# DavidSevic/gpu-nbody-simulation

Hardware: AMD Instinct MI355X
Metric: body-steps/sec (higher is better)
Workload: dtype f32

## Files before the change

### gpu-nbody-simulation_amd/csrc/bh_engine.hip

```cpp
#include "../../include/bhgpu.h"

#include <hip/hip_runtime.h>

#include <algorithm>
#include <cmath>
#include <cstdio>
#include <cstdlib>
#include <cstring>
#include <string>
#include <type_traits>
#include <vector>

#include "bh_tree.hpp"
#include "bh_walk_exact.hpp"
#include "bh_walk_f64.hpp"
#include "bh_diag.hpp"
#include "bh_direct.hpp"
#include "bh_init.hpp"
#include "bh_let.hpp"
#include "bh_migrate.hpp"
#include "bh_walk_fast.h"

using namespace bh;

#ifdef BHGPU_EXPERIMENTS
#include "../../scripts/experiments/bh_engine_hooks.hpp"
#else
struct ExpHooks {
    hipError_t create(int64_t) { return hipSuccess; }
    void walk_args(WalkFastArgs &) const {}
    void destroy(int64_t) {}
};
#endif

namespace {

thread_local std::string g_create_error;

struct DevBuf {
    void *p = nullptr;
    size_t bytes = 0;
};

}

struct bh_ctx {
    bh_config cfg{};
    int Dm = 0;
    enum class Mode { Exact, F64, Mixed, F32 };
    Mode mode = Mode::Exact;
    bool tree64() const { return mode == Mode::Exact || mode == Mode::F64; }
    bool state64() const { return mode != Mode::F32; }
    bool compat = true;
    bool exact_thresholds = false;
    int device = 0;
    hipStream_t stream = nullptr;
    bool own_stream = false;
    int64_t n = 0;
    bool uploaded = false, tree_valid = false;
    int64_t internal_cap = 0, node_cap = 0;
    int64_t bfs_max = 12288;
    int exact_bpw = 0;
    int walk_split = 0;
    bool walk_asm = true;
    int sort_bucket = 1;
    bool last_sort_bucket = false, last_sort_packed = false;
    int64_t samples_n = -1;
    uint64_t *splitters = nullptr;
    uint16_t *sort_dig = nullptr;
    int build_items = 0;
    bool hilbert = false;
    int partial_count = 0;
    double *bslots = nullptr;
    bool slots_valid = false;
    bool slots_dirty = true;

    void *pos = nullptr, *vel = nullptr, *mass = nullptr, *force = nullptr;
    void *pos2 = nullptr, *vel2 = nullptr, *mass2 = nullptr, *force2 = nullptr;
    uint32_t *orig = nullptr, *orig2 = nullptr;
    bool orig_identity = true;
    int reorder_every = 16;
    int64_t builds = 0;
    float2 *spos = nullptr;
    float4 *sstate = nullptr;
    float *smass = nullptr;
    uint64_t *keys[2] = {nullptr, nullptr};
    uint32_t *vals[2] = {nullptr, nullptr};
    uint64_t *keys_sorted = nullptr;
    uint32_t *perm = nullptr;
    uint32_t *radix_counts = nullptr, *bsum_sort = nullptr, *bsum_u32 = nullptr, *cnt = nullptr;
    uint64_t *coarse = nullptr;
    uint32_t *cell_first = nullptr;
    d3 *terms = nullptr, *bsum_d3 = nullptr;
    double *partial = nullptr, *box = nullptr;
    NodeD *gd = nullptr;
    LinkD *ld = nullptr;
    QuadF *qf = nullptr;
    NodeAux *aux = nullptr;
    int32_t *self_node = nullptr, *cell_depth = nullptr;
    uint32_t *com_pending = nullptr;
    TreeCounters *ctr = nullptr;

    int rank = 0, world = 1;
    bool let_mode = false, external_box = false;
    int64_t let_cap = 0, quads_local = 0;
    int64_t forest_base = 0;
    uint64_t *needmask = nullptr;
    uint32_t *let_tsum = nullptr, *let_outidx = nullptr;
    QuadF *let_send = nullptr;
    double *lbounds = nullptr, *all_bounds = nullptr;
    float2 *acc_part = nullptr;
    LetCounters *let_ctr = nullptr;
    int64_t *gid = nullptr;
    uint32_t *group_cost = nullptr;
    const void **walk_consts = nullptr;
    bool aux_full = false;
    bool group_cost_valid = false;
    uint32_t *body_counts = nullptr;
    double *phi = nullptr;
    uint32_t *phi_counts = nullptr;
    double *diag_part = nullptr, *diag_out = nullptr, *slots_save = nullptr;
    bool phi_current = false;
    uint32_t *slot_of = nullptr;
    int64_t *direct_targets = nullptr;
    double2 *direct_out = nullptr;
    void *check_force = nullptr;
    uint32_t *check_counts = nullptr, *check_cost = nullptr;
    TreeCounters *ctr_save = nullptr;
    bool sort_pack = true;
    unsigned long long *orb_hist = nullptr;
    double *mig_send = nullptr, *mig_recv = nullptr;
    ExpHooks exp;

    std::vector<hipEvent_t> ev;
    hipEvent_t ev_step[2] = {nullptr, nullptr}, ev_build[2] = {nullptr, nullptr};
    hipEvent_t ev_grp[3] = {nullptr, nullptr, nullptr};
    hipEvent_t ev_let[3] = {nullptr, nullptr, nullptr};
    bool let_timed = false;
    bool time_groups = false;
    int64_t steps_done = 0;
    int32_t last_nsteps = 0;
    int timed_pairs = 0;
    int64_t walk_launches = 0;
    bool step_timed = false;

    std::vector<void *> allocs;
    uint64_t device_bytes = 0;
    std::string err;
};

using Mode = bh_ctx::Mode;

namespace {

int fail(bh_ctx *c, int code, const std::string &msg)
{
    if (c) c->err = msg; else g_create_error = msg;
    return code;
}

#define BH_HIP(c, call)                                                                         \
    do {                                                                                        \
        hipError_t e_ = (call);                                                                 \
        if (e_ != hipSuccess)                                                                   \
            return fail((c), BH_ERR_DEVICE,                                                     \
                        std::string(#call) + ": " + hipGetErrorString(e_));                     \
    } while (0)

template <typename T>
int dev_alloc(bh_ctx *c, T **out, size_t count)
{
    void *p = nullptr;
    const size_t bytes = std::max<size_t>(count, 1) * sizeof(T);
    hipError_t e = hipMalloc(&p, bytes);
    if (e != hipSuccess)
        return fail(c, BH_ERR_DEVICE, std::string("hipMalloc(") + std::to_string(bytes) + "): " + hipGetErrorString(e));
    c->allocs.push_back(p);
    c->device_bytes += bytes;
    *out = static_cast<T *>(p);
    return BH_OK;
}

inline void dev_free(bh_ctx *c, void *p)
{
    if (!p) return;
    auto it = std::find(c->allocs.begin(), c->allocs.end(), p);
    if (it != c->allocs.end()) { c->allocs.erase(it); (void)hipFree(p); }
}

inline unsigned blocks_for(int64_t n, int per_block) { return (unsigned)((n + per_block - 1) / per_block); }

template <typename F>
void dispatch(F &&f) { f(); }
template <typename F, typename... B>
void dispatch(F &&f, bool b, B... rest)
{
    if (b) dispatch([&](auto... t) { f(std::true_type{}, t...); }, rest...);
    else dispatch([&](auto... t) { f(std::false_type{}, t...); }, rest...);
}

inline int64_t cell_span(const bh_ctx *c)
{
    return std::max<int64_t>(1, std::min<int64_t>(c->internal_cap, std::max<int64_t>(c->n - 1, 0) * (int64_t)std::max(1, c->Dm)));
}

void owned_range(const bh_ctx *c, int64_t *lo, int64_t *hi)
{
    if (c->let_mode) { *lo = 0; *hi = c->n; return; }
    const int64_t per = (c->n + c->world - 1) / c->world;
    const int64_t chunk = (per + kBlock - 1) / kBlock * kBlock;
    *lo = std::min<int64_t>(c->n, chunk * c->rank);
    *hi = std::min<int64_t>(c->n, chunk * (c->rank + 1));
}

constexpr int64_t kComClimbMaxBodies = 32768;
constexpr int64_t kSmallBuildBodies = 327680;
constexpr int64_t kMediumBuildBodies = 786432;
constexpr int kSmallItems = 2;

template <typename Real2, typename Real>
__global__ __launch_bounds__(kBlock) void reorder_state_kernel(uint32_t *__restrict__ perm, const Real2 *__restrict__ pos,
                                                                const Real2 *__restrict__ vel, const Real *__restrict__ mass,
                                                                const float2 *__restrict__ acc, const uint32_t *__restrict__ orig,
                                                                Real2 *__restrict__ pos2, Real2 *__restrict__ vel2,
                                                                Real *__restrict__ mass2, float2 *__restrict__ acc2,
                                                                uint32_t *__restrict__ orig2, int64_t n)
{
    const int64_t s = (int64_t)blockIdx.x * kBlock + threadIdx.x;
    if (s >= n) return;
    const uint32_t b = perm[s];
    pos2[s] = pos[b]; vel2[s] = vel[b]; mass2[s] = mass[b]; acc2[s] = acc[b];
    orig2[s] = orig ? orig[b] : b;
    perm[s] = (uint32_t)s;
}

static void launch_nodes_fast(bh_ctx *c, bool full_aux, hipStream_t st)
{
    dispatch([&](auto compat, auto full) {
        hipLaunchKernelGGL((nodes_fast_kernel<decltype(compat)::value, decltype(full)::value>), dim3(blocks_for(cell_span(c), kBlock)),
                           dim3(kBlock), 0, st, c->keys_sorted, c->coarse, c->cnt, c->cell_first, c->spos, c->smass, c->box,
                           c->terms, c->n, c->Dm, c->cfg.theta, c->internal_cap, c->qf, c->aux, c->ctr);
    }, c->compat, full_aux);
    c->aux_full = full_aux;
}

void clean_slots(bh_ctx *c)
{
    if (c->slots_dirty) hipLaunchKernelGGL(bounds_slots_reset, dim3(1), dim3(kWave), 0, c->stream, c->bslots);
    c->slots_dirty = true;
}

template <bool TREE64, bool STATE64 = TREE64, int ITEMS = kItems>
int enqueue_build_t(bh_ctx *c)
{
    constexpr int TILE = kBlock * ITEMS;
    static_assert(!TREE64 || STATE64, "an fp64 tree is built from fp64 state");
    using Real2 = typename std::conditional<STATE64, double2, float2>::type;
    using Real = typename std::conditional<STATE64, double, float>::type;
    const int64_t n = c->n;
    const int Dm = c->Dm;
    hipStream_t st = c->stream;
    const Real2 *pos = static_cast<const Real2 *>(c->pos);
    const Real *mass = static_cast<const Real *>(c->mass);

    const bool from_walk = c->slots_valid;
    double *slots = c->external_box ? nullptr : c->bslots;
    if (slots) {
        if (!from_walk) {
            const unsigned nbb = std::max(1u, std::min(1024u, blocks_for(n, kBlock)));
            clean_slots(c);
            hipLaunchKernelGGL((bounds_partial<Real2>), dim3(nbb), dim3(kBlock), 0, st, pos, n, slots);
        }
        c->slots_valid = false;
        if (n > 0) c->slots_dirty = false;
    }

    if (n > 0) {
        const bool pack = Dm >= 1 && 2 * Dm <= kPackShift && n <= ((int64_t)1 << (64 - kPackShift))
                          && c->sort_pack;
        const bool single = pack && n >= 2 && n <= 4 * kBsThreads && c->sort_bucket == 1;
        const bool bucket = !single && pack && n >= 2 && n <= kBucketMaxNBig && (c->sort_bucket == 2 || (c->sort_bucket == 1 && c->samples_n == n));
        const int nb = (n <= kBucketMaxN) ? kBuckets : kBucketsBig;
        const int ns = (nb == kBuckets) ? ((n > (int64_t)1 << 18) ? 2 * kBuckets : kBuckets)
                                        : ((n > (int64_t)3 << 20) ? kMaxSplitSamples : kBucketsBig);
        static_assert(kBucketMaxN == (int64_t)1 << 20 && kBucketMaxNBig == (int64_t)1 << 22, "BASELINE configs 3 and 4 fit");
        c->last_sort_bucket = bucket || single; c->last_sort_packed = pack;
        {
            const unsigned nkb = blocks_for(n, kBlock);
            auto keys_launch = [&](auto fs, auto pk, auto hil) {
                constexpr bool H = decltype(hil)::value, P = decltype(pk)::value, F = decltype(fs)::value;
                const bool smp = P && bucket;
                hipLaunchKernelGGL((keys_kernel<Real2, H, P, F>), dim3(nkb + (smp ? ns / kWave : 0)), dim3(kBlock), 0, st, pos, c->box,
                                   c->keys[0], c->vals[0], n, Dm, (smp && !TREE64) ? (const float2 *)c->spos : nullptr, c->splitters, nb, ns,
                                   slots, c->ctr, smp ? c->bsum_sort : nullptr, smp ? nb : 0, (smp && TREE64) ? c->perm : nullptr,
                                   from_walk ? 1 : 0);
            };
            dispatch(keys_launch, slots != nullptr, pack, c->hilbert);
        }
        if (c->time_groups) (void)hipEventRecord(c->ev_grp[0], st);
        const unsigned nbl = blocks_for(n, ITEMS == kItems ? kSortTile : TILE);
        int cur = 0;
        if (single) {
            hipLaunchKernelGGL(bucket_sort_kernel, dim3(1), dim3(kBsThreads), 0, st, c->keys[0], c->keys[1], c->vals[1],
                               nullptr, nullptr, &c->ctr->sort_spills, &c->ctr->sort_reruns, (int)n);
            cur = 1;
        } else if (bucket) {
            constexpr int SI = (ITEMS == kItems ? kSortItems : ITEMS);
            auto pass = [&](auto bits_tag) {
                constexpr int NBITS = decltype(bits_tag)::value;
                if constexpr (TREE64) {
                    hipLaunchKernelGGL((radix_hist<SI, NBITS, true>), dim3(nbl), dim3(kBlock), 0, st, c->keys[0], c->radix_counts, n,
                                       0, (int)nbl, c->splitters, c->sort_dig, nullptr);
                    hipLaunchKernelGGL(radix_rowscan, dim3(1 << NBITS), dim3(kBlock), 0, st, c->radix_counts, c->bsum_sort, (int)nbl);
                    hipLaunchKernelGGL((radix_scatter_w<SI, NBITS, 1, true, false>), dim3(nbl), dim3(kBlock), 0, st, c->keys[0], c->vals[0],
                                       c->keys[1], c->vals[1], c->radix_counts, c->bsum_sort, n, 0, (int)nbl, c->sort_dig,
                                       c->bsum_sort + kBucketStartOffset);
                } else {
                    hipLaunchKernelGGL((radix_hist<SI, NBITS, true>), dim3(nbl), dim3(kBlock), 0, st, c->keys[0], c->radix_counts, n,
                                       0, (int)nbl, c->splitters, c->sort_dig, c->bsum_sort);
                    hipLaunchKernelGGL((radix_scatter_w<SI, NBITS, 1, true>), dim3(nbl), dim3(kBlock), 0, st, c->keys[0], c->vals[0],
                                       c->keys[1], c->vals[1], c->radix_counts, c->bsum_sort, n, 0, (int)nbl, c->sort_dig,
                                       c->bsum_sort + kBucketStartOffset);
                }
            };
            if (nb == kBuckets) pass(std::integral_constant<int, 8>{}); else pass(std::integral_constant<int, 10>{});
            hipLaunchKernelGGL(bucket_sort_kernel, dim3(nb), dim3(kBsThreads), 0, st, c->keys[1], c->keys[0], c->vals[0],
                               c->bsum_sort, c->bsum_sort + kBucketStartOffset, &c->ctr->sort_spills, &c->ctr->sort_reruns, 0);
            cur = 0;
        } else {
            constexpr int SB = kSortBits, SR = 1 << SB, SI = (ITEMS == kItems ? kSortItems : ITEMS);
            const int passes = (2 * Dm + SB - 1) / SB;
            for (int p = 0; p < passes; ++p) {
                const int shift = p * SB;
                hipLaunchKernelGGL((radix_hist<SI, SB>), dim3(nbl), dim3(kBlock), 0, st, c->keys[cur], c->radix_counts, n,
                                   shift, (int)nbl);
                hipLaunchKernelGGL(radix_rowscan, dim3(SR), dim3(kBlock), 0, st, c->radix_counts, c->bsum_sort, (int)nbl);
                if (pack && p + 1 < passes)
                    hipLaunchKernelGGL((radix_scatter_w<SI, SB, 1>), dim3(nbl), dim3(kBlock), 0, st, c->keys[cur], c->vals[cur],
                                       c->keys[cur ^ 1], c->vals[cur ^ 1], c->radix_counts, c->bsum_sort, n, shift, (int)nbl);
                else if (pack)
                    hipLaunchKernelGGL((radix_scatter_w<SI, SB, 2>), dim3(nbl), dim3(kBlock), 0, st, c->keys[cur], c->vals[cur],
                                       c->keys[cur ^ 1], c->vals[cur ^ 1], c->radix_counts, c->bsum_sort, n, shift, (int)nbl);
                else
                    hipLaunchKernelGGL((radix_scatter_w<SI, SB>), dim3(nbl), dim3(kBlock), 0, st, c->keys[cur], c->vals[cur],
                                       c->keys[cur ^ 1], c->vals[cur ^ 1], c->radix_counts, c->bsum_sort, n, shift,
                                       (int)nbl);
                cur ^= 1;
            }
        }
        c->keys_sorted = c->keys[cur];
        c->perm = c->vals[cur];
        if constexpr (!TREE64) {
            if (c->reorder_every > 0 && c->builds % c->reorder_every == 0) {
                hipLaunchKernelGGL((reorder_state_kernel<Real2, Real>), dim3(blocks_for(n, kBlock)), dim3(kBlock), 0, st,
                                   c->perm, pos, static_cast<const Real2 *>(c->vel), mass,
                                   static_cast<const float2 *>(c->force), c->orig_identity ? nullptr : c->orig,
                                   static_cast<Real2 *>(c->pos2), static_cast<Real2 *>(c->vel2),
                                   static_cast<Real *>(c->mass2), static_cast<float2 *>(c->force2), c->orig2, n);
                std::swap(c->pos, c->pos2); std::swap(c->vel, c->vel2); std::swap(c->mass, c->mass2);
                std::swap(c->force, c->force2); std::swap(c->orig, c->orig2);
                c->orig_identity = false;
                pos = static_cast<const Real2 *>(c->pos);
                mass = static_cast<const Real *>(c->mass);
            }
        }
        c->builds += 1;
        if (c->time_groups) (void)hipEventRecord(c->ev_grp[1], st);

        using SReal2 = typename std::conditional<TREE64, double2, float2>::type;
        using SReal = typename std::conditional<TREE64, double, float>::type;
        auto scan_part = [&](auto si_tag) {
            constexpr int SI = decltype(si_tag)::value;
            const unsigned nbs = blocks_for(n + 1, kBlock * SI);
            hipLaunchKernelGGL((prep_kernel<TREE64, SI, Real2, Real, SReal2, SReal>), dim3(nbs), dim3(kBlock), 0, st,
                               c->keys_sorted, c->perm, pos, mass, c->cnt, c->bsum_u32, (SReal2 *)c->spos,
                               (SReal *)c->smass, c->terms, c->bsum_d3, c->coarse, n, Dm, slots);
            constexpr bool TSRC = !TREE64 && std::is_same<Real2, SReal2>::value;
            if (nbs <= 8u * kBlock) {
                hipLaunchKernelGGL((scan_apply2<TREE64, SI, true, TSRC>), dim3(nbs), dim3(kBlock), 0, st, c->cnt, c->bsum_u32,
                                   c->terms, c->bsum_d3, (int)nbs, n, c->cell_first, c->internal_cap, c->ctr,
                                   (const float2 *)c->spos, (const float *)c->smass);
            } else {
                hipLaunchKernelGGL(scan_top2, dim3(TREE64 ? 1 : 2), dim3(kBlock), 0, st, c->bsum_u32, c->bsum_d3,
                                   (int)nbs, c->ctr);
                hipLaunchKernelGGL((scan_apply2<TREE64, SI, false, TSRC>), dim3(nbs), dim3(kBlock), 0, st, c->cnt, c->bsum_u32,
                                   c->terms, c->bsum_d3, (int)nbs, n, c->cell_first, c->internal_cap, c->ctr,
                                   (const float2 *)c->spos, (const float *)c->smass);
            }
        };
        if (ITEMS == kItems && n <= (int64_t)1 << 21) scan_part(std::integral_constant<int, 4>{});
        else scan_part(std::integral_constant<int, ITEMS>{});
        c->samples_n = n;
        if (c->time_groups) (void)hipEventRecord(c->ev_grp[2], st);
    } else {
        if (slots)
            hipLaunchKernelGGL((keys_kernel<Real2, false, false, true>), dim3(1), dim3(kBlock), 0, st, pos, c->box, c->keys[0],
                               c->vals[0], n, Dm, nullptr, nullptr, 0, 0, slots, c->ctr);
        c->keys_sorted = c->keys[0];
        c->perm = c->vals[0];
        if (c->time_groups) for (auto e : c->ev_grp) (void)hipEventRecord(e, st);
    }

    if constexpr (TREE64) {
        hipLaunchKernelGGL(nodes_exact_kernel, dim3(blocks_for(cell_span(c), kBlock)), dim3(kBlock), 0, st, c->keys_sorted, c->perm,
                           c->cnt, c->cell_first, pos, mass, c->box, n, Dm, c->internal_cap, c->gd, c->ld, c->self_node,
                           c->cell_depth, c->com_pending, c->ctr, (c->mode == Mode::F64 || c->exact_thresholds) ? c->cfg.theta : 0.0,
                           c->exact_thresholds ? 1 : 0);
    } else {
        launch_nodes_fast(c, false, st);
    }
    if (TREE64 && n > 1 && c->internal_cap > 0) {
        const int64_t span = cell_span(c);
        if (n <= kComClimbMaxBodies) {
            hipLaunchKernelGGL(com_up_kernel, dim3(blocks_for(span, kBlock)), dim3(kBlock), 0, st, c->gd, c->ld,
                               c->self_node, c->com_pending, c->ctr, c->internal_cap);
        } else {
            for (int d = Dm - 1; d >= 0; --d)
                hipLaunchKernelGGL(com_level_kernel, dim3(blocks_for(span, kBlock)), dim3(kBlock), 0, st, c->gd,
                                   c->self_node, c->cell_depth, c->ctr, c->internal_cap, d);
        }
    }
    BH_HIP(c, hipGetLastError());
    c->tree_valid = true;
    return BH_OK;
}

template <int ITEMS>
static int enqueue_build_items(bh_ctx *c)
{
    if (c->tree64()) return enqueue_build_t<true, true, ITEMS>(c);
    return c->state64() ? enqueue_build_t<false, true, ITEMS>(c) : enqueue_build_t<false, false, ITEMS>(c);
}

int enqueue_build(bh_ctx *c)
{
    int items = c->build_items;
    if (items == 0) items = c->n <= kSmallBuildBodies ? 2 : c->n <= kMediumBuildBodies ? 4 : 8;
    if (c->n > (1 << 22)) items = 8;
    switch (items) {
    case 2: return enqueue_build_items<2>(c);
    case 4: return enqueue_build_items<4>(c);
    default: return enqueue_build_items<kItems>(c);
    }
}

static int fp64_bodies_per_wave(const bh_ctx *c, int64_t cnt)
{
    if (c->mode == Mode::F64 && (c->cfg.flags & BH_FLAG_WALK_NO_SPLIT)) return kWave;
    int b = 1;
    if (c->exact_bpw > 0) b = c->exact_bpw;
    else if (c->mode == Mode::F64) {
        while (b < kWave && (int64_t)b * 4096 < cnt) b <<= 1;
    } else if (cnt > 4096) {
        b = 16;
        while (b < kWave && (int64_t)b * 2048 < cnt) b <<= 1;
    }
// ... 172 lines not shown
}

int check_overflow(bh_ctx *c)
{
    TreeCounters h{};
    BH_HIP(c, hipMemcpyAsync(&h, c->ctr, sizeof(h), hipMemcpyDeviceToHost, c->stream));
    BH_HIP(c, hipStreamSynchronize(c->stream));
    if (h.overflow || (int64_t)h.n_internal > c->internal_cap)
        return fail(c, BH_ERR_CAPACITY, "tree needs " + std::to_string(1 + 4 * (int64_t)h.n_internal) +
                                        " nodes, node_capacity is " + std::to_string(c->node_cap));
    return BH_OK;
}

int new_bodies(bh_ctx *c, int64_t n)
{
    c->n = n;
    c->partial_count = 0; c->slots_valid = false;
    c->samples_n = -1;
    c->uploaded = true;
    c->tree_valid = false;
    c->steps_done = 0;
    c->orig_identity = true;
    c->builds = 0;
    c->group_cost_valid = false;
    c->phi_current = false;
    if (c->gid && n > 0) {
        hipLaunchKernelGGL(iota_i64_kernel, dim3(blocks_for(n, kBlock)), dim3(kBlock), 0, c->stream, c->gid, n);
        BH_HIP(c, hipGetLastError());
    }
    return BH_OK;
}

}

static int download_pairs(bh_ctx *c, const void *dev, double *host, int64_t count, bool is64);
static int to_caller_order(bh_ctx *c, double *host, int per);

extern "C" {

int bh_abi_version(void) { return BHGPU_ABI_VERSION; }

#ifndef BHGPU_BUILD_INFO
#define BHGPU_BUILD_INFO "digest=unknown flags=unknown"
#endif
const char *bh_build_info(void) { return BHGPU_BUILD_INFO; }

const char *bh_last_error(const bh_ctx *ctx) { return ctx ? ctx->err.c_str() : g_create_error.c_str(); }

int bh_create(const bh_config *cfg, bh_ctx **out)
{
    if (!cfg || !out) return fail(nullptr, BH_ERR_ARG, "bh_create: null argument");
    *out = nullptr;
    if (cfg->capacity < 0 || cfg->capacity > 0x7fffffffLL - 8)
        return fail(nullptr, BH_ERR_ARG, "bh_create: capacity out of range");
    if (cfg->max_depth < 1 || cfg->max_depth > 32)
        return fail(nullptr, BH_ERR_ARG, "bh_create: max_depth must be 1..32");
    if (!(cfg->theta > 0.0)) return fail(nullptr, BH_ERR_ARG, "bh_create: theta must be > 0");
    if (cfg->precision != BH_PRECISION_F64_EXACT && cfg->precision != BH_PRECISION_F32 &&
        cfg->precision != BH_PRECISION_MIXED && cfg->precision != BH_PRECISION_F64)
        return fail(nullptr, BH_ERR_ARG, "bh_create: unknown precision");
    int ndev = 0;
    if (hipGetDeviceCount(&ndev) != hipSuccess || ndev <= 0)
        return fail(nullptr, BH_ERR_NO_DEVICE, "bh_create: no HIP device (libbhgpu has no CPU fallback)");
    if (cfg->device < 0 || cfg->device >= ndev)
        return fail(nullptr, BH_ERR_ARG, "bh_create: device ordinal out of range");

    bh_ctx *c = new bh_ctx();
    c->cfg = *cfg;
    c->Dm = cfg->max_depth - 1;
    c->mode = cfg->precision == BH_PRECISION_F64_EXACT ? Mode::Exact
            : cfg->precision == BH_PRECISION_F64       ? Mode::F64
            : cfg->precision == BH_PRECISION_MIXED     ? Mode::Mixed : Mode::F32;
    c->compat = cfg->reference_compat != 0;
    c->device = cfg->device;
    if (const char *e = std::getenv("BH_WALK_SPLIT")) c->walk_split = std::atoi(e);
    if (const char *e = std::getenv("BH_EXACT_BPW")) { const int b = std::atoi(e); c->exact_bpw = (b >= 1 && b <= kWave && (b & (b - 1)) == 0) ? b : 0; }
    if (const char *e = std::getenv("BH_WALK_ASM")) c->walk_asm = std::atoi(e) != 0;
    if (const char *e = std::getenv("BH_EXACT_BFS_MAX")) c->bfs_max = std::max(0, std::atoi(e));
    c->exact_thresholds = c->mode == Mode::Exact && c->walk_asm && !(cfg->flags & BH_FLAG_WALK_PORTABLE);
    if (const char *e = std::getenv("BH_SORT_PACK")) c->sort_pack = std::atoi(e) != 0;
    if (const char *e = std::getenv("BH_SORT_BUCKET")) c->sort_bucket = std::atoi(e);
    if (const char *e = std::getenv("BH_BUILD_ITEMS")) c->build_items = std::atoi(e);
    if (const char *e = std::getenv("BH_REORDER_EVERY")) c->reorder_every = std::max(0, std::atoi(e));
    c->hilbert = !c->tree64();
    if (const char *e = std::getenv("BH_HILBERT")) c->hilbert = !c->tree64() && std::atoi(e) != 0;
    auto bail = [&](int rc) { g_create_error = c->err; bh_destroy(c); return rc; };

    if (hipSetDevice(c->device) != hipSuccess) { c->err = "hipSetDevice failed"; return bail(BH_ERR_DEVICE); }
    if (hipStreamCreateWithFlags(&c->stream, hipStreamNonBlocking) != hipSuccess) {
        c->err = "hipStreamCreate failed"; return bail(BH_ERR_DEVICE);
    }
    c->own_stream = true;

    const int64_t cap = std::max<int64_t>(cfg->capacity, 1);
    c->node_cap = cfg->node_capacity > 0 ? cfg->node_capacity : 8 * cap + 1024;
    if (c->Dm < 15) {
        int64_t full = 0, wdt = 1;
        for (int l = 0; l <= c->Dm; ++l) { full += wdt; wdt *= 4; }
        c->node_cap = std::min(c->node_cap, std::max<int64_t>(full, 1));
    }
    c->internal_cap = (c->node_cap - 1) / 4;

    const size_t rs = c->state64() ? sizeof(double) : sizeof(float);
    int rc = 0;
    auto A = [&](auto **pp, size_t count) { if (!rc) rc = dev_alloc(c, pp, count); };
    { char *t; A(&t, cap * 2 * rs); c->pos = t; }
    { char *t; A(&t, cap * 2 * rs); c->vel = t; }
    { char *t; A(&t, cap * rs); c->mass = t; }
    { char *t; A(&t, cap * 2 * (c->tree64() ? sizeof(double) : sizeof(float))); c->force = t; }
    if (!c->tree64()) {
        { char *t; A(&t, cap * 2 * rs); c->pos2 = t; }
        { char *t; A(&t, cap * 2 * rs); c->vel2 = t; }
        { char *t; A(&t, cap * rs); c->mass2 = t; }
        { char *t; A(&t, cap * 2 * sizeof(float)); c->force2 = t; }
        A(&c->orig, cap); A(&c->orig2, cap);
    }
    A(&c->keys[0], cap); A(&c->keys[1], cap); A(&c->vals[0], cap); A(&c->vals[1], cap);
    A(&c->cnt, cap + 1);
    { const size_t nbl = std::max<size_t>(blocks_for(cap, kSortTile), blocks_for(std::min<int64_t>(cap, 1 << 22), kBlock * kSmallItems));
      const size_t big = (cap > kBucketMaxN) ? (size_t)kBucketsBig * blocks_for(std::min<int64_t>(cap, kBucketMaxNBig), kBlock * kSmallItems) : 0;
      A(&c->radix_counts, std::max<size_t>((size_t)(1 << kSortBits) * nbl, big));
      A(&c->bsum_sort, 2 * kBucketStartOffset);
      A(&c->splitters, kBucketsBig);
      A(&c->sort_dig, (size_t)std::min<int64_t>(cap, kBucketMaxNBig) + 16);
    }
    const size_t scan_tiles = std::max<size_t>(blocks_for(cap + 1, kTile), blocks_for(std::min<int64_t>(cap, 1 << 22) + 1, kBlock * kSmallItems)) + 8;
    A(&c->bsum_u32, scan_tiles);
    A(&c->partial, 4 * (std::max<size_t>(1024, blocks_for(cap, kWave)) + 2));
    A(&c->box, 8); A(&c->bslots, 4 * kBoundSlots);
    A(&c->ctr, 1);
    if (c->tree64()) {
        { NodeD *g0 = nullptr; LinkD *l0 = nullptr; A(&g0, c->node_cap + 4); A(&l0, c->node_cap + 4);
          if (!rc) { c->gd = g0 + 3; c->ld = l0 + 3; } }
        A(&c->self_node, c->internal_cap + 1); A(&c->com_pending, c->internal_cap + 1); A(&c->cell_depth, c->internal_cap + 1);
        A(&c->cell_first, c->internal_cap + 1);
    } else {
        A(&c->qf, c->internal_cap + 1); A(&c->aux, 4 * (c->internal_cap + 1));
        A(&c->cell_first, c->internal_cap + 1);
        A(&c->gid, cap); A(&c->group_cost, cap / kWave + 2); A(&c->walk_consts, 4);
        A(&c->coarse, cap / 256 + 2);
        A(&c->spos, cap); A(&c->sstate, cap + 64 * kBlock + 1024); A(&c->smass, cap);
        A(&c->terms, cap + 1); A(&c->bsum_d3, scan_tiles);
    }
    if (rc) return bail(rc);
    if (hipMemset(c->ctr, 0, sizeof(TreeCounters)) != hipSuccess) { c->err = "hipMemset failed"; return bail(BH_ERR_DEVICE); }
    if (!c->tree64()) {
        const void *wc[4] = {c->aux, c->spos, c->smass, nullptr};
        if (hipMemcpy(c->walk_consts, wc, sizeof(wc), hipMemcpyHostToDevice) != hipSuccess) { c->err = "hipMemcpy failed"; return bail(BH_ERR_DEVICE); }
    }
    if (!c->tree64() && c->exp.create(cap) != hipSuccess) { c->err = "experiment hooks: allocation failed"; return bail(BH_ERR_DEVICE); }
    auto create = [](auto &evs) { for (auto &e : evs) if (hipEventCreate(&e) != hipSuccess) return false; return true; };
    if (!create(c->ev_step) || !create(c->ev_build) || !create(c->ev_grp) || !create(c->ev_let)) {
        c->err = "hipEventCreate failed"; return bail(BH_ERR_DEVICE);
    }
    *out = c;
    return BH_OK;
}

void bh_destroy(bh_ctx *c)
{
    if (!c) return;
    (void)hipSetDevice(c->device);
    if (c->stream) (void)hipStreamSynchronize(c->stream);
    c->exp.destroy(c->n);
    for (void *p : c->allocs) (void)hipFree(p);
    auto destroy = [](auto &evs) { for (auto e : evs) if (e) (void)hipEventDestroy(e); };
// ... 1058 lines not shown
```

### gpu-nbody-simulation_amd/csrc/bh_tree.hpp

```cpp
#pragma once

#include <type_traits>

#include "bh_prims.hpp"
#include "bh_sort.hpp"
#include "bh_nodes.hpp"
#include "bh_bounds.hpp"

namespace bh {

constexpr int kCoarse = 256;

__device__ __forceinline__ int shared_levels(uint64_t a, uint64_t b, int Dm)
{
    const uint64_t x = a ^ b;
    if (x == 0) return Dm;
    return (__clzll((long long)x) - (64 - 2 * Dm)) >> 1;
}

template <typename Real2>
__global__ __launch_bounds__(kBlock) void bounds_partial(const Real2 *__restrict__ pos, int64_t n, double *slots)
{
    double xlo = INFINITY, xhi = -INFINITY, ylo = INFINITY, yhi = -INFINITY;
    for (int64_t i = (int64_t)blockIdx.x * kBlock + threadIdx.x; i < n; i += (int64_t)gridDim.x * kBlock) {
// ... 46 lines not shown
            if (bx) x0 = mx; else x1 = mx;
            if (by) y0 = my; else y1 = my;
        }
    } else {
        for (int l = 0; l < Dm; ++l) {
            const double mx = (x0 + x1) / 2, my = (y0 + y1) / 2;
            const int c = pick_child(x, y, mx, my);
            if (HILBERT) {
                k = (k << 2) | (uint64_t)hilbert_digit(state, c);
                state = hilbert_next(state, c);
            } else {
                k = (k << 2) | (uint64_t)c;
            }
            descend(c, mx, my, x0, x1, y0, y1);
        }
    }
    return k;
}

__device__ __forceinline__ uint32_t hilbert3_entry(uint32_t t)
{
    int state = (int)(t >> 6);
    const uint32_t iy3 = (t >> 3) & 7u, ix3 = t & 7u;
    uint32_t digits = 0;
#pragma unroll
    for (int l = 2; l >= 0; --l) {
        const int c = (int)(((ix3 >> l) & 1u) | (((iy3 >> l) & 1u) << 1));
        digits = (digits << 2) | (uint32_t)hilbert_digit(state, c);
        state = hilbert_next(state, c);
    }
    return ((uint32_t)state << 6) | digits;
}

template <bool HILBERT>
__device__ __forceinline__ uint64_t key_of_fast(double x, double y, double x0, double x1, double y0, double y1, int Dm,
                                                double scale_x, double scale_y, double margin_x, double margin_y,
                                                const uint8_t *hil3 = nullptr)
{
    const double side = (double)(1u << Dm);
    const double tx = (x - x0) * scale_x, ty = (y - y0) * scale_y;
    const double fx = floor(tx), fy = floor(ty);
    const double rx = tx - fx, ry = ty - fy;
    const bool sure = rx > margin_x && rx < 1.0 - margin_x && ry > margin_y && ry < 1.0 - margin_y &&
                      fx >= 0.0 && fx < side && fy >= 0.0 && fy < side;
    if (!sure) return key_of<HILBERT>(x, y, x0, x1, y0, y1, Dm);
    const uint32_t ix = (uint32_t)fx, iy = (uint32_t)fy;
    uint64_t k = 0;
    int state = 0;
    int l = Dm - 1;
    if (HILBERT && hil3 != nullptr) {
        for (; (l + 1) % 3 != 0; --l) {
            const int c = (int)(((ix >> l) & 1u) | (((iy >> l) & 1u) << 1));
            k = (k << 2) | (uint64_t)hilbert_digit(state, c);
            state = hilbert_next(state, c);
        }
        uint32_t st = (uint32_t)state;
        for (; l >= 2; l -= 3) {
            const uint32_t e = hil3[(st << 6) | (((iy >> (l - 2)) & 7u) << 3) | ((ix >> (l - 2)) & 7u)];
            k = (k << 6) | (uint64_t)(e & 63u);
            st = e >> 6;
        }
        return k;
    }
    if (!HILBERT) {
        auto spread = [](uint32_t v) -> uint64_t {
            uint64_t u = v;
            u = (u | (u << 16)) & 0x0000FFFF0000FFFFull;
            u = (u | (u << 8)) & 0x00FF00FF00FF00FFull;
            u = (u | (u << 4)) & 0x0F0F0F0F0F0F0F0Full;
            u = (u | (u << 2)) & 0x3333333333333333ull;
            u = (u | (u << 1)) & 0x5555555555555555ull;
            return u;
        };
        return spread(ix) | (spread(iy) << 1);
    }
    for (; l >= 0; --l) {
        const int c = (int)(((ix >> l) & 1u) | (((iy >> l) & 1u) << 1));
        k = (k << 2) | (uint64_t)hilbert_digit(state, c);
        state = hilbert_next(state, c);
    }
    return k;
}

template <typename Real2, bool HILBERT, bool PACK = false, bool FROM_SLOTS = false>
__global__ __launch_bounds__(kBlock) void keys_kernel(const Real2 *__restrict__ pos,
                                                       double *box_global,
                                                       uint64_t *__restrict__ keys,
                                                       uint32_t *__restrict__ idx, int64_t n, int Dm,
                                                       const float2 *__restrict__ samples = nullptr,
                                                       uint64_t *__restrict__ splitters = nullptr, int nb = 0,
                                                       int ns = 0, double *slots = nullptr, TreeCounters *ctr = nullptr,
                                                       uint32_t *__restrict__ zero_words = nullptr, int n_zero = 0,
                                                       const uint32_t *__restrict__ sample_perm = nullptr, int from_walk = 0)
{
    if (blockIdx.x == 0)
        for (int k = threadIdx.x; k < n_zero; k += kBlock) zero_words[k] = 0u;
    __shared__ double s_box[FROM_SLOTS ? 8 : 1];
    __shared__ int s_keep;
    if (FROM_SLOTS) {
        if (threadIdx.x < kWave) {
            const double *sl = slots + 4 * threadIdx.x;
            const double xlo = wave_min(sl[0]), xhi = wave_max(sl[1]), ylo = wave_min(sl[2]), yhi = wave_max(sl[3]);
            const bool keep = from_walk && xlo > xhi;
            if (threadIdx.x == 0) s_keep = keep ? 1 : 0;
            if (threadIdx.x < 2) {
                const int a = threadIdx.x;
                if (keep) {
                    s_box[2 * a] = box_global[2 * a]; s_box[2 * a + 1] = box_global[2 * a + 1];
                    s_box[4 + a] = box_global[4 + a]; s_box[6 + a] = box_global[6 + a];
                } else {
                    const double ex = xhi - xlo, ey = yhi - ylo;
                    const double span = (ex < ey) ? ey : ex;
                    double pad = 0.1 * span;
                    if (span == 0.0) pad = 1e-6;
                    s_box[2 * a] = (a ? ylo : xlo) - pad; s_box[2 * a + 1] = (a ? yhi : xhi) + pad;
                    write_key_consts_axis(s_box, a, Dm);
                }
            }
        }
        __syncthreads();
        if (blockIdx.x == 0 && threadIdx.x == 0) {
            if (!s_keep) {
#pragma unroll
                for (int k = 0; k < 8; ++k) box_global[k] = s_box[k];
                ctr->overflow = 0;
            }
            ctr->n_internal = 0;
            ctr->visits = 0; ctr->interactions = 0; ctr->wave_nodes = 0; ctr->wave_quads = 0; ctr->wave_accepts = 0;
        }
    }
    double x0, x1, y0, y1, bk4, bk5, bk6, bk7;
    if (FROM_SLOTS) {
        x0 = s_box[0]; x1 = s_box[1]; y0 = s_box[2]; y1 = s_box[3]; bk4 = s_box[4]; bk5 = s_box[5]; bk6 = s_box[6]; bk7 = s_box[7];
    } else {
        x0 = box_global[0]; x1 = box_global[1]; y0 = box_global[2]; y1 = box_global[3];
        bk4 = box_global[4]; bk5 = box_global[5]; bk6 = box_global[6]; bk7 = box_global[7];
    }
    const int nsb = (samples != nullptr || sample_perm != nullptr) ? ns / kWave : 0;
    if ((int)blockIdx.x < nsb) {
        __shared__ uint64_t sk[kMaxSplitSamples];
        const int t = threadIdx.x;
        const int Ds = Dm, lg_ns = 31 - __clz(ns), lg_os = lg_ns - (31 - __clz(nb));
        const double side = (double)(1u << Ds), top = side - 1.0, down = 1.0 / (double)(1u << (Dm - Ds));
        const double sx = (bk4 > 0.0) ? bk4 * down : side / (x1 - x0), sy = (bk5 > 0.0) ? bk5 * down : side / (y1 - y0);
        float2 qs[kMaxSplitSamples / kBlock];
#pragma unroll
        for (int k = 0; k < kMaxSplitSamples / kBlock; ++k) {
            const int j = t + k * kBlock;
            qs[k] = float2{0.f, 0.f};
            if (j < ns) {
                const int64_t rk = ((int64_t)j * n) >> lg_ns;
                if (sample_perm != nullptr) { const Real2 pp = pos[sample_perm[rk]]; qs[k] = float2{(float)pp.x, (float)pp.y}; }
                else qs[k] = samples[rk];
            }
        }
#pragma unroll
        for (int k = 0; k < kMaxSplitSamples / kBlock; ++k) {
            const int j = t + k * kBlock;
            if (j >= ns) break;
            uint64_t mine = 0;
            if (j > 0) {
                const float2 q = qs[k];
                const double fx = fmin(fmax(((double)q.x - x0) * sx, 0.0), top);
                const double fy = fmin(fmax(((double)q.y - y0) * sy, 0.0), top);
                const uint32_t ix = (uint32_t)(int)fx, iy = (uint32_t)(int)fy;
                int state = 0;
                for (int l = Ds - 1; l >= 0; --l) {
                    const int cc = (int)(((ix >> l) & 1u) | (((iy >> l) & 1u) << 1));
                    mine = (mine << 2) | (uint64_t)(HILBERT ? hilbert_digit(state, cc) : cc);
                    state = hilbert_next(state, cc);
                }
            }
            sk[j] = (mine << 11) | (uint64_t)j;
        }
        __syncthreads();
        const int sidx = (int)blockIdx.x * kWave + (t >> 2), part = t & 3, span = ns >> 2;
        const uint64_t tagged = sk[sidx];
        int rank = 0;
#pragma unroll 16
        for (int q = part * span; q < (part + 1) * span; ++q) rank += (sk[q] < tagged) ? 1 : 0;
        rank += __shfl_xor(rank, 1);
        rank += __shfl_xor(rank, 2);
        if (part == 0 && (rank & ((1 << lg_os) - 1)) == 0) splitters[rank >> lg_os] = tagged >> 11;
        return;
    }
    __shared__ uint8_t s_hil3[HILBERT ? 256 : 1];
    if (HILBERT) {
        static_assert(kBlock == 256, "one table entry per thread");
        s_hil3[threadIdx.x] = (uint8_t)hilbert3_entry(threadIdx.x);
        __syncthreads();
    }
    const int64_t i = ((int64_t)blockIdx.x - nsb) * kBlock + threadIdx.x;
    if (i >= n) return;
    const uint64_t k = key_of_fast<HILBERT>((double)pos[i].x, (double)pos[i].y, x0, x1, y0, y1, Dm, bk4, bk5, bk6, bk7,
                                            HILBERT ? s_hil3 : nullptr);
    if (PACK) {
        keys[i] = k | ((uint64_t)i << kPackShift);
    } else {
        keys[i] = k;
        idx[i] = (uint32_t)i;
    }
}

template <bool EXACT, int ITEMS, typename Real2, typename Real, typename SReal2 = Real2, typename SReal = Real>
__global__ __launch_bounds__(kBlock) void prep_kernel(const uint64_t *__restrict__ keys,
                                                       const uint32_t *__restrict__ perm,
                                                       const Real2 *__restrict__ pos,
                                                       const Real *__restrict__ mass,
                                                       uint32_t *__restrict__ cnt,
                                                       uint32_t *__restrict__ bsum_u32,
                                                       SReal2 *__restrict__ spos, SReal *__restrict__ smass,
                                                       d3 *__restrict__ terms, d3 *__restrict__ bsum_d3,
                                                       uint64_t *__restrict__ coarse, int64_t n, int Dm,
                                                       double *slots_reset = nullptr)
{
    if (slots_reset != nullptr && blockIdx.x == 0 && threadIdx.x < kBoundSlots) {
        double *w = slots_reset + 4 * threadIdx.x;
        w[0] = INFINITY; w[1] = -INFINITY; w[2] = INFINITY; w[3] = -INFINITY;
    }
    __shared__ uint32_t smu[kWavesPerBlock + 1];
    __shared__ d3 smd[kWavesPerBlock + 1];
    const int64_t base = (int64_t)blockIdx.x * (kBlock * ITEMS);
    uint32_t csum = 0;
    d3 tsum{0.0, 0.0, 0.0};
#pragma unroll
    for (int k = 0; k < ITEMS; ++k) {
        const int64_t i = base + k * kBlock + threadIdx.x;
        if (i < n) {
            uint32_t c = 0;
            if (i + 1 < n) {
                const uint64_t kc = keys[i];
                const int L = shared_levels(kc, keys[i + 1], Dm);
                const int Lp = (i == 0) ? -1 : shared_levels(keys[i - 1], kc, Dm);
                const int hi = (L < Dm - 1) ? L : Dm - 1;
                c = (hi > Lp) ? (uint32_t)(hi - Lp) : 0u;
            }
            cnt[i] = c;
            csum += c;
            if (!EXACT && (i & (kCoarse - 1)) == 0) coarse[i / kCoarse] = keys[i];
            if (!EXACT) {
                const uint32_t b = perm[i];
                const Real2 p = pos[b];
                const Real m = mass[b];
                spos[i] = SReal2{static_cast<SReal>(p.x), static_cast<SReal>(p.y)};
                smass[i] = static_cast<SReal>(m);
                const d3 t{(double)m, (double)m * (double)p.x, (double)m * (double)p.y};
                if (!std::is_same<Real2, SReal2>::value) terms[i] = t;
                tsum += t;
            }
        } else if (!EXACT && i == n) {
            if (!std::is_same<Real2, SReal2>::value) terms[n] = d3{0.0, 0.0, 0.0};
        }
    }
    uint32_t utot;
    (void)block_exclusive_sum(csum, smu, utot);
    if (threadIdx.x == 0) bsum_u32[blockIdx.x] = utot;
    if (!EXACT) {
        d3 dtot;
        (void)block_exclusive_sum(tsum, smd, dtot);
        if (threadIdx.x == 0) bsum_d3[blockIdx.x] = dtot;
    }
}

__global__ __launch_bounds__(kBlock) void scan_top2(uint32_t *__restrict__ bsum_u32,
                                                     d3 *__restrict__ bsum_d3, int nb,
                                                     TreeCounters *ctr)
{
    if (blockIdx.x == 0) {
        __shared__ uint32_t sm[kWavesPerBlock + 1];
        uint32_t carry = 0;
        for (int c0 = 0; c0 < nb; c0 += kBlock) {
            const int i = c0 + threadIdx.x;
            const uint32_t v = (i < nb) ? bsum_u32[i] : 0u;
            uint32_t tot;
            const uint32_t ex = block_exclusive_sum(v, sm, tot);
            if (i < nb) bsum_u32[i] = carry + ex;
            carry += tot;
        }
        if (threadIdx.x == 0) ctr->n_internal = carry;
    } else {
        __shared__ d3 sm[kWavesPerBlock + 1];
        d3 carry{0.0, 0.0, 0.0};
        for (int c0 = 0; c0 < nb; c0 += kBlock) {
            const int i = c0 + threadIdx.x;
            const d3 v = (i < nb) ? bsum_d3[i] : d3{0.0, 0.0, 0.0};
            d3 tot;
            const d3 ex = block_exclusive_sum(v, sm, tot);
            if (i < nb) bsum_d3[i] = carry + ex;
            carry += tot;
        }
    }
}

template <bool EXACT, int ITEMS, bool FOLD, bool TSRC = false>
__global__ __launch_bounds__(kBlock) void scan_apply2(uint32_t *__restrict__ cnt,
                                                       const uint32_t *__restrict__ bsum_u32,
                                                       d3 *__restrict__ terms,
                                                       const d3 *__restrict__ bsum_d3, int nbs, int64_t n,
                                                       uint32_t *__restrict__ cell_first,
                                                       int64_t internal_cap, TreeCounters *ctr,
                                                       const float2 *__restrict__ spos = nullptr,
                                                       const float *__restrict__ smass = nullptr)
{
    __shared__ uint32_t smu[kWavesPerBlock + 1];
    __shared__ d3 smd[kWavesPerBlock + 1];
    const int64_t base = (int64_t)blockIdx.x * (kBlock * ITEMS);
    uint32_t ucarry;
    d3 dcarry{0.0, 0.0, 0.0};
    if (FOLD) {
        uint32_t vb = 0, va = 0;
        d3 db{0.0, 0.0, 0.0};
        for (int t = threadIdx.x; t < nbs; t += kBlock) {
            const uint32_t v = bsum_u32[t];
            va += v;
            if (t < (int)blockIdx.x) {
                vb += v;
                if (!EXACT) db += bsum_d3[t];
            }
        }
        uint32_t uall;
        (void)block_exclusive_sum(vb, smu, ucarry);
        (void)block_exclusive_sum(va, smu, uall);
        if (blockIdx.x == 0 && threadIdx.x == 0) ctr->n_internal = uall;
        if (!EXACT) (void)block_exclusive_sum(db, smd, dcarry);
    } else {
        ucarry = bsum_u32[blockIdx.x];
// ... 216 lines not shown

    if (d == 0) {
        const double ex = x1 - x0, ey = y1 - y0;
        gd[0].size = size_slot((ex > ey) ? ex : ey);
        ld[0] = LinkD{quad, -1};
        self_node[0] = 0;
    }
    cell_depth[r] = d;
    uint32_t n_sub = 0;
    int64_t bc4[4], nc4[4];
    uint32_t bi1[4], offc[4];
    uint64_t kprev[4], kcur[4];
    bool sub4[4], one4[4];
#pragma unroll
    for (int c = 0; c < 4; ++c) {
        bc4[c] = b[c]; nc4[c] = b[c + 1] - b[c];
        sub4[c] = nc4[c] > 1 && d + 1 < Dm;
        one4[c] = nc4[c] == 1 && d + 1 < Dm;
        bi1[c] = one4[c] ? perm[bc4[c]] : 0u;
        offc[c] = sub4[c] ? off[bc4[c]] : 0u;
        kcur[c] = sub4[c] ? keys[bc4[c]] : 0ull;
        kprev[c] = (sub4[c] && bc4[c] > 0) ? keys[bc4[c] - 1] : 0ull;
    }
    double m1[4];
    double2 p1[4];
#pragma unroll
    for (int c = 0; c < 4; ++c) {
        m1[c] = one4[c] ? mass[bi1[c]] : 0.0;
        p1[c] = one4[c] ? pos[bi1[c]] : double2{0.0, 0.0};
    }
#pragma unroll
    for (int c = 0; c < 4; ++c) {
        const double cx0 = (c & 1) ? mx : x0, cx1 = (c & 1) ? x1 : mx;
        const double cy0 = (c & 2) ? my : y0, cy1 = (c & 2) ? y1 : my;
        const double ex = cx1 - cx0, ey = cy1 - cy0;
        const double size = (ex > ey) ? ex : ey;
        const int64_t bc = bc4[c], nc = nc4[c];
        const int32_t node = quad + c;
        double m = 0.0, cx = 0.0, cy = 0.0;
        int32_t child = -1, occ = -1;
        if (nc == 0) {
        } else if (d + 1 == Dm) {
            for (int64_t j = bc; j < bc + nc; ++j) {
                const uint32_t bi = perm[j];
                const double bm = mass[bi], bx = pos[bi].x, by = pos[bi].y;
                cx = (m * cx + bm * bx) / (m + bm);
                cy = (m * cy + bm * by) / (m + bm);
                m += bm;
            }
            occ = (nc == 1) ? (-(int32_t)perm[bc] - 2) : -1;
        } else if (nc == 1) {
            m = m1[c]; cx = p1[c].x; cy = p1[c].y;
            occ = (int32_t)bi1[c];
        } else {
            const int Lpc = (bc == 0) ? -1 : shared_levels(kprev[c], kcur[c], Dm);
            const uint32_t rc = offc[c] + (uint32_t)((d + 1) - (Lpc + 1));
            child = 1 + 4 * (int32_t)rc;
            self_node[rc] = node;
            ++n_sub;
        }
        double *sn = s_nd + threadIdx.x * 16 + 4 * c;
        sn[0] = cx; sn[1] = cy; sn[2] = m; sn[3] = size_slot(size);
        s_ln[threadIdx.x * 8 + 2 * c] = child; s_ln[threadIdx.x * 8 + 2 * c + 1] = occ;
    }
    pending[r] = n_sub;
    }
    __syncthreads();
    {
        const int64_t left = (int64_t)total - r_block;
        const int cells = (left < kBlock) ? (int)left : kBlock;
        double2 *dn = reinterpret_cast<double2 *>(gd + 1 + 4 * r_block);
        const double2 *sn = reinterpret_cast<const double2 *>(s_nd);
        for (int k = threadIdx.x; k < cells * 8; k += kBlock) dn[k] = sn[k];
        int2 *dl = reinterpret_cast<int2 *>(ld + 1 + 4 * r_block);
        const int2 *sl = reinterpret_cast<const int2 *>(s_ln);
        for (int k = threadIdx.x; k < cells * 4; k += kBlock) dl[k] = sl[k];
    }
}

constexpr int kMaxBucket = 1024;
constexpr int kKeyHalo = 768;
constexpr int kKeyWin = kBlock + 1 + kKeyHalo;

template <bool COMPAT, bool FULL_AUX = false>
__global__ __launch_bounds__(kBlock, 5) void nodes_fast_kernel(
    const uint64_t *__restrict__ keys, const uint64_t *__restrict__ coarse,
    const uint32_t *__restrict__ off, const uint32_t *__restrict__ cell_first,
    const float2 *__restrict__ spos,
    const float *__restrict__ smass, const double *__restrict__ box, const d3 *__restrict__ psum,
    int64_t n64, int Dm, double theta, int64_t internal_cap, QuadF *__restrict__ qf,
    NodeAux *__restrict__ aux, TreeCounters *ctr)
{
    constexpr int kStageBytes = kBlock * (FULL_AUX ? 28 : 20) * 4, kWinBytes = kKeyWin * 8;
    __shared__ __attribute__((aligned(16))) unsigned char lds_raw[kStageBytes > kWinBytes ? kStageBytes : kWinBytes];
    uint64_t *wkeys = reinterpret_cast<uint64_t *>(lds_raw);
    __shared__ int32_t s_wlo;
    __shared__ double s_thr0;
    int32_t *stage_q = reinterpret_cast<int32_t *>(lds_raw);
    int32_t *stage_a = stage_q + kBlock * 20;
    const int32_t n = (int32_t)n64;
    const uint32_t total = ctr->n_internal;
    float *qw = reinterpret_cast<float *>(qf);
    int32_t *qi = reinterpret_cast<int32_t *>(qf);
    auto put = [&](int32_t quad, int slot, float cx, float cy, float m, float thr, int32_t child) {
        const int64_t o = (int64_t)quad * 20;
        qw[o + 2 * slot] = cx; qw[o + 2 * slot + 1] = cy; qw[o + 8 + slot] = m; qw[o + 12 + slot] = thr;
        qi[o + 16 + slot] = child;
    };
    auto put_lds = [&](int slot, float cx, float cy, float m, float thr, int32_t child) {
        int32_t *o = stage_q + threadIdx.x * 20;
        o[2 * slot] = __float_as_int(cx); o[2 * slot + 1] = __float_as_int(cy);
        o[8 + slot] = __float_as_int(m); o[12 + slot] = __float_as_int(thr); o[16 + slot] = child;
    };

    if (total == 0) {
        if (blockIdx.x == 0 && threadIdx.x == 0) {
            for (int k = 0; k < 4; ++k) { put(0, k, 0.f, 0.f, 0.f, -1.f, -1); aux[k] = NodeAux{0, 0}; }
            if (n >= 1) {
                const d3 t = psum[n];
                const bool one = (n == 1);
                const float cx = one ? spos[0].x : (float)(t.b / t.a), cy = one ? spos[0].y : (float)(t.c / t.a);
                const float m = (t.a > 1e-15) ? (one ? smass[0] : (float)t.a) : 0.f;
                const bool bucket = (n > 1) && (n <= kMaxBucket) && !COMPAT;
                put(0, 0, cx, cy, m, bucket ? INFINITY : 0.f, bucket ? -2 : -1);
                aux[0] = NodeAux{0, (int32_t)n};
            }
        }
        return;
    }
    if ((int64_t)total > internal_cap) {
        if (blockIdx.x == 0 && threadIdx.x == 0) ctr->overflow = 1;
        return;
    }
    const uint32_t r_block = blockIdx.x * kBlock;
    if (r_block >= total) return;

    const uint32_t r = r_block + threadIdx.x;
    const int32_t i_pre = (r < total) ? (int32_t)cell_first[r] : 0;
    const uint32_t off_pre = (r < total) ? off[i_pre] : 0u;

    if (threadIdx.x == 0) {
        s_wlo = i_pre - 1;
        const double ex0 = box[1] - box[0], ey0 = box[3] - box[2];
        const double q0 = ((ex0 > ey0) ? ex0 : ey0) / theta;
        s_thr0 = q0 * q0;
    }
    __syncthreads();
    const int32_t wlo = s_wlo;
    for (int k = threadIdx.x; k < kKeyWin; k += kBlock) {
        const int32_t j = wlo + k;
        wkeys[k] = (j >= 0 && j < n) ? keys[j] : 0ull;
    }
    __syncthreads();
    auto K = [&](int32_t j) -> uint64_t {
        const int32_t k = j - wlo;
        const bool in = (uint32_t)k < (uint32_t)kKeyWin;
        uint64_t v = wkeys[in ? k : 0];
        if (__ballot(!in) != 0ull) {
            asm volatile("" : "+v"(v));
            if (!in) v = keys[j];
        }
        return v;
    };

    auto search = [&](auto nt_tag, auto keyfn, int32_t lo0, int32_t hi0, int sh, const uint64_t *target, int32_t *res) {
        constexpr int NT = decltype(nt_tag)::value;
        int32_t lo[NT], hi[NT];
#pragma unroll
// ... 299 lines not shown
```

Before: 2.373 billion.

## Fuse periodic state reorder into prep kernel and batch keys per thread

After: 2.380 billion, median of 2. Within noise of the previous version (+0.3%).

```diff
diff --git a/gpu-nbody-simulation_amd/csrc/bh_engine.hip b/gpu-nbody-simulation_amd/csrc/bh_engine.hip
--- a/gpu-nbody-simulation_amd/csrc/bh_engine.hip
+++ b/gpu-nbody-simulation_amd/csrc/bh_engine.hip
@@ -80,6 +80,8 @@
     uint32_t *orig = nullptr, *orig2 = nullptr;
     bool orig_identity = true;
     int reorder_every = 16;
+    bool reorder_fused = true;
+    int keys_items = 0;
     int64_t builds = 0;
     float2 *spos = nullptr;
     float4 *sstate = nullptr;
@@ -217,6 +219,7 @@
 constexpr int64_t kSmallBuildBodies = 327680;
 constexpr int64_t kMediumBuildBodies = 786432;
 constexpr int kSmallItems = 2;
+constexpr int64_t kKeysItemsBodies = 524288;
 
 template <typename Real2, typename Real>
 __global__ __launch_bounds__(kBlock) void reorder_state_kernel(uint32_t *__restrict__ perm, const Real2 *__restrict__ pos,
@@ -286,16 +289,26 @@
         static_assert(kBucketMaxN == (int64_t)1 << 20 && kBucketMaxNBig == (int64_t)1 << 22, "BASELINE configs 3 and 4 fit");
         c->last_sort_bucket = bucket || single; c->last_sort_packed = pack;
         {
-            const unsigned nkb = blocks_for(n, kBlock);
-            auto keys_launch = [&](auto fs, auto pk, auto hil) {
+            auto keys_launch = [&](auto fs, auto pk, auto hil, auto items_tag) {
                 constexpr bool H = decltype(hil)::value, P = decltype(pk)::value, F = decltype(fs)::value;
+                constexpr int KI = F ? decltype(items_tag)::value : 1;
+                const unsigned nkb = blocks_for(n, kBlock * KI);
                 const bool smp = P && bucket;
-                hipLaunchKernelGGL((keys_kernel<Real2, H, P, F>), dim3(nkb + (smp ? ns / kWave : 0)), dim3(kBlock), 0, st, pos, c->box,
+                hipLaunchKernelGGL((keys_kernel<Real2, H, P, F, KI>), dim3(nkb + (smp ? ns / kWave : 0)), dim3(kBlock), 0, st, pos, c->box,
                                    c->keys[0], c->vals[0], n, Dm, (smp && !TREE64) ? (const float2 *)c->spos : nullptr, c->splitters, nb, ns,
                                    slots, c->ctr, smp ? c->bsum_sort : nullptr, smp ? nb : 0, (smp && TREE64) ? c->perm : nullptr,
                                    from_walk ? 1 : 0);
             };
-            dispatch(keys_launch, slots != nullptr, pack, c->hilbert);
+            auto with_items = [&](auto items_tag) {
+                dispatch([&](auto fs, auto pk, auto hil) { keys_launch(fs, pk, hil, items_tag); }, slots != nullptr, pack, c->hilbert);
+            };
+            const int ki = c->keys_items ? c->keys_items : (n >= kKeysItemsBodies ? 2 : 1);
+            switch (ki) {
+            case 2: with_items(std::integral_constant<int, 2>{}); break;
+            case 4: with_items(std::integral_constant<int, 4>{}); break;
+            case 8: with_items(std::integral_constant<int, 8>{}); break;
+            default: with_items(std::integral_constant<int, 1>{}); break;
+            }
         }
         if (c->time_groups) (void)hipEventRecord(c->ev_grp[0], st);
         const unsigned nbl = blocks_for(n, ITEMS == kItems ? kSortTile : TILE);
@@ -350,8 +363,11 @@
         }
         c->keys_sorted = c->keys[cur];
         c->perm = c->vals[cur];
+        bool reorder_in_prep = false;
         if constexpr (!TREE64) {
-            if (c->reorder_every > 0 && c->builds % c->reorder_every == 0) {
+            const bool reorder = c->reorder_every > 0 && c->builds % c->reorder_every == 0;
+            reorder_in_prep = reorder && c->reorder_fused;
+            if (reorder && !reorder_in_prep) {
                 hipLaunchKernelGGL((reorder_state_kernel<Real2, Real>), dim3(blocks_for(n, kBlock)), dim3(kBlock), 0, st,
                                    c->perm, pos, static_cast<const Real2 *>(c->vel), mass,
                                    static_cast<const float2 *>(c->force), c->orig_identity ? nullptr : c->orig,
@@ -372,6 +388,23 @@
         auto scan_part = [&](auto si_tag) {
             constexpr int SI = decltype(si_tag)::value;
             const unsigned nbs = blocks_for(n + 1, kBlock * SI);
+            if constexpr (!TREE64) {
+                if (reorder_in_prep) {
+                    const ReorderArgs<Real2, Real> ro{static_cast<const Real2 *>(c->vel), static_cast<const float2 *>(c->force),
+                                                      c->orig_identity ? nullptr : c->orig, static_cast<Real2 *>(c->pos2),
+                                                      static_cast<Real2 *>(c->vel2), static_cast<Real *>(c->mass2),
+                                                      static_cast<float2 *>(c->force2), c->orig2};
+                    hipLaunchKernelGGL((prep_kernel<false, SI, Real2, Real, SReal2, SReal, true>), dim3(nbs), dim3(kBlock), 0, st,
+                                       c->keys_sorted, c->perm, pos, mass, c->cnt, c->bsum_u32, (SReal2 *)c->spos,
+                                       (SReal *)c->smass, c->terms, c->bsum_d3, c->coarse, n, Dm, slots, ro);
+                    std::swap(c->pos, c->pos2); std::swap(c->vel, c->vel2); std::swap(c->mass, c->mass2);
+                    std::swap(c->force, c->force2); std::swap(c->orig, c->orig2);
+                    c->orig_identity = false;
+                    pos = static_cast<const Real2 *>(c->pos);
+                    mass = static_cast<const Real *>(c->mass);
+                }
+            }
+            if (!reorder_in_prep)
             hipLaunchKernelGGL((prep_kernel<TREE64, SI, Real2, Real, SReal2, SReal>), dim3(nbs), dim3(kBlock), 0, st,
                                c->keys_sorted, c->perm, pos, mass, c->cnt, c->bsum_u32, (SReal2 *)c->spos,
                                (SReal *)c->smass, c->terms, c->bsum_d3, c->coarse, n, Dm, slots);
@@ -710,6 +743,8 @@
     if (const char *e = std::getenv("BH_SORT_BUCKET")) c->sort_bucket = std::atoi(e);
     if (const char *e = std::getenv("BH_BUILD_ITEMS")) c->build_items = std::atoi(e);
     if (const char *e = std::getenv("BH_REORDER_EVERY")) c->reorder_every = std::max(0, std::atoi(e));
+    if (const char *e = std::getenv("BH_REORDER_FUSED")) c->reorder_fused = std::atoi(e) != 0;
+    if (const char *e = std::getenv("BH_KEYS_ITEMS")) { const int k = std::atoi(e); c->keys_items = (k == 1 || k == 2 || k == 4 || k == 8) ? k : 0; }
     c->hilbert = !c->tree64();
     if (const char *e = std::getenv("BH_HILBERT")) c->hilbert = !c->tree64() && std::atoi(e) != 0;
     auto bail = [&](int rc) { g_create_error = c->err; bh_destroy(c); return rc; };
diff --git a/gpu-nbody-simulation_amd/csrc/bh_tree.hpp b/gpu-nbody-simulation_amd/csrc/bh_tree.hpp
--- a/gpu-nbody-simulation_amd/csrc/bh_tree.hpp
+++ b/gpu-nbody-simulation_amd/csrc/bh_tree.hpp
@@ -152,7 +152,7 @@
     return k;
 }
 
-template <typename Real2, bool HILBERT, bool PACK = false, bool FROM_SLOTS = false>
+template <typename Real2, bool HILBERT, bool PACK = false, bool FROM_SLOTS = false, int ITEMS = 1>
 __global__ __launch_bounds__(kBlock) void keys_kernel(const Real2 *__restrict__ pos,
                                                        double *box_global,
                                                        uint64_t *__restrict__ keys,
@@ -260,19 +260,40 @@
         s_hil3[threadIdx.x] = (uint8_t)hilbert3_entry(threadIdx.x);
         __syncthreads();
     }
-    const int64_t i = ((int64_t)blockIdx.x - nsb) * kBlock + threadIdx.x;
-    if (i >= n) return;
-    const uint64_t k = key_of_fast<HILBERT>((double)pos[i].x, (double)pos[i].y, x0, x1, y0, y1, Dm, bk4, bk5, bk6, bk7,
-                                            HILBERT ? s_hil3 : nullptr);
-    if (PACK) {
-        keys[i] = k | ((uint64_t)i << kPackShift);
-    } else {
-        keys[i] = k;
-        idx[i] = (uint32_t)i;
-    }
-}
-
-template <bool EXACT, int ITEMS, typename Real2, typename Real, typename SReal2 = Real2, typename SReal = Real>
+    const int64_t base = ((int64_t)blockIdx.x - nsb) * (kBlock * ITEMS) + threadIdx.x;
+    Real2 q[ITEMS];
+#pragma unroll
+    for (int k = 0; k < ITEMS; ++k) {
+        const int64_t i = base + k * kBlock;
+        q[k] = (i < n) ? pos[i] : Real2{0, 0};
+    }
+#pragma unroll
+    for (int k = 0; k < ITEMS; ++k) {
+        const int64_t i = base + k * kBlock;
+        if (i >= n) break;
+        const uint64_t key = key_of_fast<HILBERT>((double)q[k].x, (double)q[k].y, x0, x1, y0, y1, Dm, bk4, bk5, bk6, bk7,
+                                                  HILBERT ? s_hil3 : nullptr);
+        if (PACK) {
+            keys[i] = key | ((uint64_t)i << kPackShift);
+        } else {
+            keys[i] = key;
+            idx[i] = (uint32_t)i;
+        }
+    }
+}
+
+template <typename Real2, typename Real>
+struct ReorderArgs {
+    const Real2 *vel = nullptr;
+    const float2 *acc = nullptr;
+    const uint32_t *orig = nullptr;
+    Real2 *pos2 = nullptr, *vel2 = nullptr;
+    Real *mass2 = nullptr;
+    float2 *acc2 = nullptr;
+    uint32_t *orig2 = nullptr;
+};
+
+template <bool EXACT, int ITEMS, typename Real2, typename Real, typename SReal2 = Real2, typename SReal = Real, bool REORDER = false>
 __global__ __launch_bounds__(kBlock) void prep_kernel(const uint64_t *__restrict__ keys,
                                                        const uint32_t *__restrict__ perm,
                                                        const Real2 *__restrict__ pos,
@@ -282,8 +303,10 @@
                                                        SReal2 *__restrict__ spos, SReal *__restrict__ smass,
                                                        d3 *__restrict__ terms, d3 *__restrict__ bsum_d3,
                                                        uint64_t *__restrict__ coarse, int64_t n, int Dm,
-                                                       double *slots_reset = nullptr)
-{
+                                                       double *slots_reset = nullptr,
+                                                       const ReorderArgs<Real2, Real> ro = {})
+{
+    static_assert(!(EXACT && REORDER), "the exact modes keep their state in caller order");
     if (slots_reset != nullptr && blockIdx.x == 0 && threadIdx.x < kBoundSlots) {
         double *w = slots_reset + 4 * threadIdx.x;
         w[0] = INFINITY; w[1] = -INFINITY; w[2] = INFINITY; w[3] = -INFINITY;
@@ -312,6 +335,13 @@
                 const uint32_t b = perm[i];
                 const Real2 p = pos[b];
                 const Real m = mass[b];
+                if constexpr (REORDER) {
+                    const Real2 v = ro.vel[b];
+                    const float2 a = ro.acc[b];
+                    const uint32_t o = ro.orig ? ro.orig[b] : b;
+                    ro.pos2[i] = p; ro.vel2[i] = v; ro.mass2[i] = m; ro.acc2[i] = a; ro.orig2[i] = o;
+                    const_cast<uint32_t *>(perm)[i] = (uint32_t)i;
+                }
                 spos[i] = SReal2{static_cast<SReal>(p.x), static_cast<SReal>(p.y)};
                 smass[i] = static_cast<SReal>(m);
                 const d3 t{(double)m, (double)m * (double)p.x, (double)m * (double)p.y};
@@ -694,8 +724,12 @@
 constexpr int kKeyHalo = 768;
 constexpr int kKeyWin = kBlock + 1 + kKeyHalo;
 
+#ifndef BH_NODES_FAST_WGS
+#define BH_NODES_FAST_WGS 5
+#endif
+constexpr int kNodesFastWgs = BH_NODES_FAST_WGS;
 template <bool COMPAT, bool FULL_AUX = false>
-__global__ __launch_bounds__(kBlock, 5) void nodes_fast_kernel(
+__global__ __launch_bounds__(kBlock, kNodesFastWgs) void nodes_fast_kernel(
     const uint64_t *__restrict__ keys, const uint64_t *__restrict__ coarse,
     const uint32_t *__restrict__ off, const uint32_t *__restrict__ cell_first,
     const float2 *__restrict__ spos,
```
